# exosports/BART

Hardware: AMD Instinct MI355X
Metric: forward spectra/sec (100 layers x 1e4 wavenumbers) (higher is better)
Workload: dtype f64; 1 GPU; H2O+CO+CO2+CH4 eclipse, 100 layers x 10000 wavenumbers, 10 walkers batched per GPU per step (BASELINE config 3), opacity-table path, 27 T planes, H2-H2 CIA, 5 ray angles, toomuch 10, SURVEY 8d opacities, every step its own profile preparation; nlayers=100, nwave=10000, integ=1, cut=slant, cia_interp=spline, kappa_model=survey8d, parallelism=single GPU

## Files before the change

### bart_amd/csrc/capi.hip

```cpp
#include <cstring>
#include <stdexcept>
#include <string>

#include "../../include/bartrt.h"
#include "comm.hpp"
#include "contrib.hpp"
#include "engine.hpp"
#include "lbl.hpp"
#include "share.hpp"
#include "step.hpp"
#include "rt_launch.hpp"
#include "rtc.hpp"
#include "svc.hpp"

#include <climits>
#include <cstdio>
#include <cstdlib>

#include <sys/stat.h>
#include <unistd.h>

using namespace bartrt;

static Engine *g_eng = nullptr;
// ... 596 lines not shown
  return BARTRT_OK;
}

int bartrt_walked_end(int *walked, int cap, int *nwalkers, int *ncolumns, int *wn_per_column,
                      char *kernel, int kernel_len) {
  NEED_ENGINE();
  return guarded([&] {
    Engine *e = g_eng;
    e->want_walked = false;
    HIPCHK(hipDeviceSynchronize());
    const int n = e->walked_nwalkers, nc = e->walked_info.ncolumns;
    if (nwalkers) *nwalkers = n;
    if (ncolumns) *ncolumns = nc;
    if (wn_per_column) *wn_per_column = e->walked_info.wn_per_column;
    if (kernel && kernel_len > 0) {
      std::snprintf(kernel, (size_t)kernel_len, "%s%s%s%s", e->walked_info.kernel, e->walked_info.rtc ? " [instantiated at run time]" : "",
                    e->walked_info.prep_folded ? " [prepares its own walkers]" : "",
                    e->walked_info.window ? " [table through a moving window]" : "");
    }
    if (walked && n > 0) {
      if ((size_t)cap < (size_t)n * nc) throw std::invalid_argument("walked_end: buffer too small");
      HIPCHK(hipMemcpy(walked, e->d_walked, sizeof(int) * (size_t)n * nc, hipMemcpyDeviceToHost));
    }
    return BARTRT_OK;
  });
}

int bartrt_get_rtc_stats(int *available, int *compiled, int *from_disk, int *failed, double *compile_seconds) {
  const RtcStats st = rtc_stats();
  if (available) *available = rtc_available() ? 1 : 0;
  if (compiled) *compiled = st.compiled;
// ... 302 lines not shown
```

### bart_amd/csrc/engine.hip

```cpp
#include "engine.hpp"
#include "lbl.hpp"
#include "lds.hpp"
#include "prep.hpp"
#include "contrib.hpp"
#include "share.hpp"
#include "step.hpp"
#include "svc.hpp"

#include <algorithm>
#include <climits>
#include <cmath>
#include <cstdlib>
#include <cstring>
#include <stdexcept>

#include <sys/stat.h>
#include <unistd.h>

namespace bartrt {

EngineStream::~EngineStream() {
  for (auto e : ev) (void)hipEventDestroy(e);
  if (stream) (void)hipStreamDestroy(stream);
}
// ... 183 lines not shown
      hi_wn = 1.0 / (cfg_num(cfg, "wllow", 0) * wlfct);
    } else {
      throw IoError{"transit cfg: no spectral range (wnlow/wnhigh or wllow/wlhigh)"};
    }
    double d = cfg_num(cfg, "wndelt", 1.0) * wnfct;
    if (!(d > 0) || !(hi_wn > lo_wn)) throw IoError{"transit cfg: bad spectral sampling"};
    long n = (long)std::floor((hi_wn - lo_wn) / d + 1e-9) + 1;
    wn_full.resize(n);
    for (long i = 0; i < n; i++) wn_full[i] = lo_wn + d * (double)i;
    M = 0; Nt = 2; tgrid = {0.0, 1.0};
  }
  Wfull = (int)wn_full.size();
  lo = (int)((long)Wfull * shard_rank / shard_n);
  hi = (int)((long)Wfull * (shard_rank + 1) / shard_n);
  if (hi <= lo) throw IoError{"--shard leaves this rank without wavenumber samples"};
}

void Engine::read_geometry() {
  angles = cfg_list(cfg, "raygrid");
  if (angles.empty()) angles = {0, 20, 40, 60, 80};
  A = (int)angles.size();
  if (A > kMaxAngles) throw IoError{"raygrid: too many angles"};
  for (int a = 0; a < A; a++)
    if (angles[a] < 0 || angles[a] >= 90 || (a && angles[a] <= angles[a - 1]))
      throw IoError{"raygrid: angles must increase within [0, 90)"};
  toomuch = cfg_num(cfg, "toomuch", 20.0);
  if (!cfg_has(cfg, "gsurf") || !cfg_has(cfg, "refpress") || !cfg_has(cfg, "refradius"))
    throw IoError{"transit cfg: gsurf, refpress and refradius are required"};
  gsurf = cfg_num(cfg, "gsurf", 0);
  refpress = cfg_num(cfg, "refpress", 0) * 1e6;
// ... 230 lines not shown
  }
  pa.consts = d_prep_consts;
  if (M > kMaxMol) throw IoError{"more opacity-table molecules than the kernels are built for (16)"};
  for (int m = 0; m < M; m++) pa.opmol[m] = opmol[m];
  pa.ncia_temps = (int)cia_temp.size();
  const size_t prep_lds = sizeof(double) * prep_lds_doubles(L, S, Nt, pa.ncia_temps);
  if (prep_lds > kLdsMax)
    throw IoError{"the column's preparation does not fit in LDS: L = " + std::to_string(L) + " layers and S = " +
                  std::to_string(S) + " species need " + std::to_string(prep_lds) + " bytes of the " +
                  std::to_string(kLdsMax) + " a workgroup has"};
  pa.iH2 = iH2; pa.iHe = iHe;

  RtArgs &r = rt;
  r.L = L; r.M = M; r.Nt = Nt; r.C = C; r.A = A; r.W = Wl; r.Wfull = Wfull;
  r.kappa = d_kappa; r.cia = d_cia; r.wn = d_wn;
  r.kappa_bytes = (unsigned long long)L * Nt * M * Wl * 8ull;
  r.cia_bytes = (unsigned long long)cia_planes.size() * 8ull;
  for (int a = 0; a < A; a++) {
    double lo_a = a == 0 ? 0.0 : 0.5 * (angles[a - 1] + angles[a]);
    double hi_a = a == A - 1 ? 90.0 : 0.5 * (angles[a] + angles[a + 1]);
    double sl = std::sin(lo_a * kPI / 180.0), sh = std::sin(hi_a * kPI / 180.0);
    r.wgt[a] = kPI * (sh * sh - sl * sl);
    r.invmu[a] = 1.0 / std::cos(angles[a] * kPI / 180.0);
    r.wq[a] = r.wgt[a] * r.invmu[a];
    r.mu[a] = std::cos(angles[a] * kPI / 180.0);
  }
}

void Engine::start_workspaces() {
  if (!cfg_has(cfg, "opacityfile") && cfg_has(cfg, "linedb")) {
// ... 15 lines not shown
    }
  HIPCHK(hipMemcpy(d_prof, hp.data(), sizeof(double) * hp.size(), hipMemcpyHostToDevice));
  run(RunRequest(d_prof, 1, d_spec, rec[0].ok, stream));
  run(RunRequest(d_prof, nw, d_spec, rec[0].ok, stream));
  HIPCHK(hipStreamSynchronize(stream));
  forget_profiles();
}

void Engine::setup(const TCfg &cfg_in, int shard_rank, int shard_n) {
  cfg = cfg_in;
  read_settings();
  generate_missing_opacity_file(shard_rank);
  read_atmosphere();
  OpacityHeader oh;
  read_grid(oh, shard_rank, shard_n);
  read_geometry();
  open_device();
  upload_table(oh);
  std::vector<double> cia_planes, cia_temp;
  resample_cia(cia_planes, cia_temp);
  upload_constants(cia_planes, cia_temp);
  start_workspaces();
}

void Engine::ensure_walkers(int n) {
  if (n <= cap_walkers) return;
  int cap = std::max(n, cap_walkers * 2);
  HIPCHK(hipDeviceSynchronize());
  if (last_prof == d_prof) forget_profiles();
  pf_have_prof = nullptr;
  if (cap2) {
    rec[1].reserve((size_t)cap, L, M, C);
    cap2 = cap;
  }
  d_prof.reserve((size_t)cap * (S + 1) * L);
  rec[0].reserve((size_t)cap, L, M, C);
  d_spec.reserve((size_t)cap * W());
  d_rad.reserve((size_t)cap * L);
  if (solution == 1) {
    d_rtop.reserve((size_t)cap * L);
    d_ds.reserve((size_t)cap * chord_table_size(L));
  }
  cap_walkers = cap;
}

void Engine::ensure_second_set() {
  if (cap2 >= cap_walkers) return;
  HIPCHK(hipDeviceSynchronize());
  rec[1].reserve((size_t)cap_walkers, L, M, C);
  cap2 = cap_walkers;
}

void Engine::wait(hipStream_t st) {
  if (!sync_poll || !h_flag) { HIPCHK(hipStreamSynchronize(st)); return; }
  const unsigned int want = ++flag_seq;
  HIPCHK(hipStreamWriteValue32(st, d_flag, want, 0));
  volatile unsigned int *f = h_flag;
  long spins = 0;
  while (*f != want) {
    __builtin_ia32_pause();
    if ((++spins & 0xfffff) == 0 && hipStreamQuery(st) != hipErrorNotReady) { HIPCHK(hipStreamSynchronize(st)); break; }
  }
  __atomic_thread_fence(__ATOMIC_ACQUIRE);
}
// ... 126 lines not shown

PrepArgs Engine::prep_args(const RunRequest &rq, const RecordSet &records) {
  PrepArgs pa = prep;
  pa.nwalkers = rq.n;
  pa.prof = rq.prof;
  pa.gsurf = gsurf; pa.refradius = refradius;
  pa.scat_flag = rq.scat_flag >= 0 ? rq.scat_flag : scat_flag; pa.scat_value = scat_value;
  pa.has_cloud = has_cloud; pa.cloudtop = cloudtop;
  pa.cloud_rup = cloud_rup; pa.cloud_rdown = cloud_rdown; pa.cloud_ext = cloud_ext;
  pa.coef = records.coef; pa.idx = records.idx; pa.kstop = records.kstop;
  pa.ok = rq.ok ? rq.ok : rec[0].ok.get();
  pa.rad_out = d_rad;
  pa.over = rq.over;
  pa.rtop = solution == 1 ? d_rtop.get() : nullptr;
  pa.ds = solution == 1 ? d_ds.get() : nullptr;
  return pa;
}

static int rt_block() {
  static const int b = [] { const char *e = std::getenv("BARTRT_BLOCK"); return e ? std::atoi(e) : 64; }();
  return (b == 128 || b == 256) ? b : 64;
}

RtArgs Engine::rt_args(const RunRequest &rq, const PrepArgs &pa, const Prefetch &pf, bool eclipse_rt, bool timed) {
  const int n = rq.n, block = rt_block();
  RtArgs r = rt;
  r.nwalkers = n;
  r.nsel = rq.sel_walkers > n ? rq.sel_walkers : 0;
  if (kernel_by_local) r.Wfull = r.W;
  r.coef = pa.coef; r.idx = pa.idx; r.kstop = pa.kstop;
// ... 55 lines not shown
    r.walked_out = d_walked;
    walked_nwalkers = n;
  }
  return r;
}

void Engine::run_chunk(const RunRequest &rq) {
  const int n = rq.n;
  hipStream_t st = rq.stream;
  if (n > cap_walkers) ensure_walkers(n);
  const bool eclipse_rt = solution == 0 && !rq.lbl_fused;
  const bool plain = eclipse_rt && !lbl && !rq.d_ext && !rq.prep_hook && !rq.want_tau && !rq.want_intens;
  const bool pf_ok = plain && !rq.over;
  const Prefetch pf = plan_prefetch(pf_ok, rq);
  const bool use_have = pf.have, want_next = pf.want_next;
  const PrepArgs pa = prep_args(rq, rec[pf.bset]);
  const bool try_fold = plain && !use_have && !want_next && std::max(n, rq.sel_walkers) <= 4 && integ == 1 && cut_slant &&
                        A == 5;
  if (use_have) {
    if (rq.ok) HIPCHK(hipMemcpyAsync(rq.ok, rec[pf.bset].ok, (size_t)n, hipMemcpyDeviceToDevice, st));
  } else if (rq.prep_hook) HIPCHK(rq.prep_hook(pa, st, rq.prep_hook_ctx));
  else if (!try_fold) HIPCHK(launch_prep(pa, st));
  if (solution == 1) HIPCHK(launch_chord_table(pa, st));

  const bool timed = timing && n > 0 && rt.W > 0 && (timing_seen++ % timing_stride == 0);
  const RtArgs r = rt_args(rq, pa, pf, eclipse_rt, timed);
  if (rq.lbl_fused) lbl_rt_eclipse(*this, rq.prof, n, r, st);
  else if (solution == 1) {
    RtLaunchInfo li;
    HIPCHK(launch_transit(r, st, &li));
    if (want_walked) walked_info = li;
  }
  else {
    RtLaunchInfo li;
    bool folded = false;
    if (try_fold) HIPCHK(launch_rt_folded(r, pa, rt_block(), st, &li, &folded));
    if (!folded) {
      if (try_fold) HIPCHK(launch_prep(pa, st));
      li = RtLaunchInfo{};
      HIPCHK(launch_rt(r, rt_block(), st, &li));
    }
    if (want_walked) walked_info = li;
    if (want_next && li.prep_fused) {
      pf_have_prof = rq.next_prof; pf_have_n = rq.next_n; pf_have_buf = 1 - pf.bset;
      pf_have_stream = st; pf_have_set = pf.now;
    }
  }
  if (timed) {
    if (rq.lbl_fused) HIPCHK(hipEventRecord(ev[ev_used + 1], st));
    ev_used += 2;
  }
}

}
```

### bart_amd/csrc/engine.hpp

```cpp
#pragma once
#include <hip/hip_runtime.h>

#include <string>
#include <vector>

#include "devbuf.hpp"
#include "io.hpp"
#include "kernels.hpp"

namespace bartrt {

hipError_t launch_prep(const PrepArgs &a, hipStream_t st);
hipError_t launch_rt(const RtArgs &a, int block, hipStream_t st, RtLaunchInfo *info = nullptr);
hipError_t launch_rt_folded(const RtArgs &a, const PrepArgs &prep, int block, hipStream_t st, RtLaunchInfo *info, bool *folded);
hipError_t launch_transit(const RtArgs &a, hipStream_t st, RtLaunchInfo *info = nullptr);
hipError_t launch_chord_table(const PrepArgs &a, hipStream_t st);
hipError_t launch_grid_transpose(const double *src, double *dst, long planes, int M, int W, hipStream_t st);

int parse_integ(const std::string &v);
int resolve_share_mode(const TCfg &cfg, bool no_service);

struct TableShare;
struct StepArgs;
struct Lbl;
struct Comm;
struct CfState;

struct EngineStream {
  hipStream_t stream = nullptr;
  std::vector<hipEvent_t> ev;
  ~EngineStream();
};

struct RecordSet {
  DevBuf<double> coef;
  DevBuf<idx_t> idx;
  DevBuf<int> kstop;
  DevBuf<unsigned char> ok;
  void reserve(size_t cap, int L, int M, int C) {
    coef.reserve(cap * L * coef_stride(M, C));
    idx.reserve(cap * L * idx_stride(C));
    kstop.reserve(cap);
    ok.reserve(cap);
  }
};

struct RunRequest {
  const double *prof;
  int n;
  double *spec;
  unsigned char *ok;
  hipStream_t stream;
  bool want_tau = false;
// ... 14 lines not shown
struct Engine : EngineStream {
  TCfg cfg;
  Atm atm;
  MolInfo mol;
  int L = 0, S = 0, M = 0, Nt = 0, C = 0, A = 0;
  int Wfull = 0, lo = 0, hi = 0;
  int W() const { return hi - lo; }
  std::vector<double> wn_full, tgrid, mass, angles;
  std::vector<int> opmol;
  double toomuch = 20.0, gsurf = 0, refpress = 0, refradius = 0;
  int scat_flag = 0, iH2 = -1, iHe = -1, has_cloud = 0;
  int solution = 0;
  int integ = 0;
  bool cut_slant = false;
  bool kernel_by_local = true;
  bool cia_spline = false;
  double starrad = 0;
  double scat_value = 0, cloudtop = 0;
  double cloud_rup = 0, cloud_rdown = 0, cloud_ext = 0;
  bool transparent = false;
  int device = 0;
  const double *d_kappa = nullptr;
  DevBuf<double> kappa_own, d_cia, d_wn, d_wn_full, d_press, d_mass, d_diam;
  TableShare *kappa_share = nullptr;
  int share_mode = -1;
  DevBuf<double> d_prep_consts;
  PrepArgs prep{};
  RtArgs rt{};
  int cap_walkers = 0;
  DevBuf<double> d_prof, d_spec;
// ... 43 lines not shown
  PrepSettings pf_have_set{};
  int cap2 = 0;
  DevBuf<char> d_slog;
  StepArgs *step = nullptr;
  Lbl *lbl = nullptr;
  CfState *cf = nullptr;

  ~Engine();
  void init(int argc, const char **argv);
  void setup(const TCfg &cfg_in, int shard_rank, int shard_n);
  void read_settings();
  void generate_missing_opacity_file(int shard_rank);
  void read_atmosphere();
  void read_grid(OpacityHeader &oh, int shard_rank, int shard_n);
  void read_geometry();
  void open_device();
  void upload_table(const OpacityHeader &oh);
  void resample_cia(std::vector<double> &cia_planes, std::vector<double> &cia_temp);
  void upload_constants(const std::vector<double> &cia_planes, const std::vector<double> &cia_temp);
  void start_workspaces();
  void ensure_walkers(int n);
  void ensure_second_set();
  void ensure_pin(size_t bytes);
  void run(const RunRequest &rq);
  void run_host(const double *prof, int n, int nprof, double *spec, int nwave, unsigned char *ok);
  void run_chunks(const RunRequest &rq, int chunk, bool with_ext);
  void run_chunk(const RunRequest &rq);
  struct Prefetch;
  Prefetch plan_prefetch(bool pf_ok, const RunRequest &rq);
  PrepArgs prep_args(const RunRequest &rq, const RecordSet &records);
// ... 8 lines not shown
```

### bart_amd/csrc/kernels.hip

```cpp
#include "integ.hpp"
#include "kernels.hpp"
#include "lds.hpp"
#include "prep.hpp"

#include <cmath>
#include <cstdio>
#include <cstdlib>
#include <cstring>
#include <utility>

namespace bartrt {

template <int INTEG>
bool launch_rt_spec(const RtArgs &a, int block, hipStream_t st, KernelMode mode, bool force_window,
                    bool allow_sq, hipError_t &err, RtLaunchInfo *info, const PrepArgs *fold = nullptr);
extern template bool launch_rt_spec<0>(const RtArgs &, int, hipStream_t, KernelMode, bool, bool, hipError_t &, RtLaunchInfo *, const PrepArgs *);
extern template bool launch_rt_spec<1>(const RtArgs &, int, hipStream_t, KernelMode, bool, bool, hipError_t &, RtLaunchInfo *, const PrepArgs *);
extern template bool launch_rt_spec<2>(const RtArgs &, int, hipStream_t, KernelMode, bool, bool, hipError_t &, RtLaunchInfo *, const PrepArgs *);

__global__ __launch_bounds__(256) void prep_profiles(PrepArgs p) {
  extern __shared__ double sm[];
  prep_block(p, blockIdx.x, sm);
}

__device__ inline void block_to_work_g(int b, int nwalkers, int &tile, int &walker) {
  const int xcd = b & 7, j = b >> 3;
  walker = j % nwalkers;
  tile = (j / nwalkers) * 8 + xcd;
}

template <int AT, int MT, int CT, int INTEG>
__global__ __launch_bounds__(256) void rt_eclipse(RtArgs p) {
  extern __shared__ double smem[];
  const int A = AT > 0 ? AT : p.A;
  const int M = MT >= 0 ? MT : p.M;
  const int C = CT >= 0 ? CT : p.C;
// ... 131 lines not shown
}

hipError_t launch_grid_transpose(const double *src, double *dst, long planes, int M, int W, hipStream_t st) {
  if (planes <= 0 || M <= 0 || W <= 0) return hipSuccess;
  const int ntiles = (W + 63) / 64;
  if (planes * ntiles > 0x7fffffffL) return hipErrorInvalidValue;
  hipLaunchKernelGGL(grid_transpose, dim3((unsigned)(planes * ntiles)), dim3(64), 0, st, src, dst, M, W, ntiles);
  return hipGetLastError();
}

hipError_t launch_prep(const PrepArgs &a, hipStream_t st) {
  if (a.nwalkers <= 0) return hipSuccess;
  const size_t sh = sizeof(double) * prep_lds_doubles(a.L, a.S, a.Nt, a.ncia_temps);
  static size_t allowed = kLdsDefault;
  if (hipError_t e = allow_lds(prep_profiles, sh, allowed); e != hipSuccess) return e;
  hipLaunchKernelGGL(prep_profiles, dim3(a.nwalkers), dim3(256), sh, st, a);
  return hipGetLastError();
}

template <int AT, int INTEG>
static hipError_t launch_rt_t(const RtArgs &a, int block, int nblocks, hipStream_t st) {
  const size_t sh = sizeof(double) * ((size_t)a.L * coef_stride(a.M, a.C) +
                                      (INTEG == kIntegSimpson ? simpson_lds_doubles(a.L) : 0)) +
                    sizeof(idx_t) * (size_t)a.L * idx_stride(a.C);
  static size_t allowed = 64 * 1024;
  if (sh > allowed) {
    if (sh > 160 * 1024) return hipErrorInvalidValue;
    hipError_t e = hipFuncSetAttribute(reinterpret_cast<const void *>(rt_eclipse<AT, -1, -1, INTEG>),
                                       hipFuncAttributeMaxDynamicSharedMemorySize, (int)sh);
    if (e != hipSuccess) return e;
    allowed = sh;
// ... 76 lines not shown
```

### bart_amd/csrc/kernels.hpp

```cpp
#pragma once
#ifndef __HIPCC_RTC__
#include <hip/hip_runtime.h>
#include <hip/hip_ext.h>
#include <cstdint>
#else
typedef struct ihipEvent_t *hipEvent_t;
namespace std {
template <class T, T v> struct integral_constant { static constexpr T value = v; using value_type = T; constexpr operator T() const { return v; } };
using true_type = integral_constant<bool, true>;
using false_type = integral_constant<bool, false>;
template <bool B, class T, class F> struct conditional { using type = T; };
template <class T, class F> struct conditional<false, T, F> { using type = F; };
template <bool B, class T, class F> using conditional_t = typename conditional<B, T, F>::type;
}
#endif

#define BARTRT_MC_LIST(X) \
  X(1, 0) X(1, 1) X(1, 2) X(2, 0) X(2, 1) X(2, 2) X(3, 0) X(3, 1) X(3, 2) X(4, 0) X(4, 1) X(4, 2) \
  X(5, 0) X(5, 1) X(5, 2) X(6, 0) X(6, 1) X(6, 2)                                                 \
  X(1, 4) X(2, 4) X(3, 4) X(4, 4) X(5, 4) X(6, 4)
#define BARTRT_QADJ_LIST(X) BARTRT_MC_LIST(X)
#define BARTRT_EXT_C_LIST(X) X(0) X(1) X(2) X(4)

#define BARTRT_RT_LAUNCH(kernel, grid, block, sh, st, args) \
// ... 102 lines not shown
  int ref_ib;
  double ref_f;
  double ref_lnp;
  double gsurf, refradius;
  int scat_flag, iH2, iHe, has_cloud;
  double scat_value, cloudtop;
  double cloud_rup, cloud_rdown, cloud_ext;
  const double *over;
  double *coef;
  idx_t *idx;
  int *kstop;
  unsigned char *ok;
  double *rad_out;
  double *rtop;
  double *ds;
};

struct RtArgs {
  int L, M, Nt, C, A, W, nwalkers, ntiles;
  int nsel;
  int Wfull;
  const double *kappa;
  const double *cia;
  unsigned long long kappa_bytes, cia_bytes;
  int window;
  const double *ext;
  const double *wn;
  const double *coef;
  const idx_t *idx;
  const int *kstop;
// ... 8 lines not shown
  double thr[kMaxAngles];
  double thrb[kMaxAngles];
  int drank[kMaxAngles];
  void *slog;
  double *spec;
  double *tau_out;
  int *last_out;
  double *intens_out;
  int *walked_out;
  const double *rtop, *ds;
  double inv_starrad2;
  int transparent;
  hipEvent_t ev_start, ev_stop;
  int nprep;
  PrepArgs prep_next;
};
__host__ __device__ inline int prep_slots(int nprep) { return (nprep + 7) / 8 * 8; }

inline void slant_thresholds(RtArgs &r) {
  for (int a = 0; a < r.A; a++) {
    const double im = r.invmu[a];
    double t = r.toomuch / im;
    if (!(t == t) || t > 1.7e308 || t < 0.0) { r.thr[a] = t < 0.0 ? -1.0 : 1.7976931348623157e308; continue; }
    for (int it = 0; it < 64 && t * im > r.toomuch; it++) t = __builtin_nextafter(t, 0.0);
    for (int it = 0; it < 64; it++) {
      const double up = __builtin_nextafter(t, 1.7976931348623157e308);
      if (up == t || up * im > r.toomuch) break;
      t = up;
    }
    r.thr[a] = t;
// ... 6 lines not shown
    r.drank[a] = rk;
  }
}
inline size_t slant_log_bytes(int nwalkers, int ntiles, int block, int A) {
  return (size_t)nwalkers * (size_t)ntiles * (size_t)block * (size_t)A * 20u;
}

struct RtLaunchInfo {
  const char *kernel = "";
  int wn_per_column = 64;
  int ncolumns = 0;
  bool prep_fused = false;
  bool prep_folded = false;
  bool rtc = false;
  bool window = false;
};

#ifndef __HIPCC_RTC__
enum class KernelMode { kDefault, kGeneric, kMono, kMonoOcc, kMonoIlp, kSplit, kQuad, kOcto, kHexa, kR32, kAdj8, kAdj16 };
KernelMode rt_kernel_mode();
#endif

constexpr double kExpShift = 6755399441055744.0;
constexpr double kExpMin = -708.0;

__device__ __forceinline__ double exp_scale(double p, double shifted) {
  const int hi = __double2hiint(p) + (__double2loint(shifted) << 20);
  return __hiloint2double(hi, __double2loint(p));
}

// ... 5 lines not shown
  double p = 2.5110037605963777e-08;
  p = fma(p, r, 2.763263963904103e-07);
  p = fma(p, r, 2.755724091857897e-06);
  p = fma(p, r, 2.4801485482328494e-05);
  p = fma(p, r, 0.00019841269890047113);
  p = fma(p, r, 0.0013888888952314775);
  p = fma(p, r, 0.008333333333319601);
  p = fma(p, r, 0.0416666666664881);
  p = fma(p, r, 0.1666666666666668);
  p = fma(p, r, 0.5000000000000019);
  p = fma(p, r, 1.0);
  p = fma(p, r, 1.0);
  return exp_scale(p, t);
}

__device__ __forceinline__ double rcp_core(double d) {
  double y = __builtin_amdgcn_rcp(d);
  double e = fma(-d, y, 1.0);
  y = fma(y, e, y);
  e = fma(-d, y, 1.0);
  return fma(y, e, y);
}
__device__ __forceinline__ double rcp_n1(double d) {
  const double y = __builtin_amdgcn_rcp(d);
  return fma(y, fma(-d, y, 1.0), y);
}

template <int N>
__device__ __forceinline__ void exp_rt_n(const double (&x)[N], double (&out)[N]) {
  double t[N], r[N], q[N];
// ... 115 lines not shown
```

### bart_amd/csrc/prep.hpp

```cpp
#pragma once
#include "kernels.hpp"

#ifdef BARTRT_PHASE_CLOCK
extern __device__ unsigned long long g_phase_clock[32];
#define BARTRT_PHASE(n) do { if (blockIdx.x == 0 && threadIdx.x == 0) g_phase_clock[n] = __builtin_amdgcn_s_memrealtime(); } while (0)
#else
#define BARTRT_PHASE(n) do {} while (0)
#endif

namespace bartrt {

__device__ inline int bracket_dev(const double *g, const double *ginv, int n, double t) {
  if (n <= 2) return 0;
  double x = (t - g[0]) * ginv[0];
  int j = x > 0.0 ? (x < (double)(n - 2) ? (int)x : n - 2) : 0;
  const double a = g[j], b = g[j + 1];
  if ((j == n - 2 || b > t) && (j == 0 || a <= t)) return j;
  while (j < n - 2 && g[j + 1] <= t) j++;
  while (j > 0 && g[j] > t) j--;
  return j;
}


__host__ __device__ inline size_t prep_lds_doubles(int L, int S, int Nt, int ncia_temps) {
// ... 202 lines not shown
  if (threadIdx.x == 0) {
    int ks = L - 1;
    if (has_cloud) {
      for (int k = 0; k < L; k++)
        if (sPress[L - 1 - k] >= cloudtop) { ks = k | kDeckBit; break; }
    }
    if (fold.kstop) *fold.kstop = ks;
    if (fold.global) {
      p.kstop[w] = ks;
      if (p.ok) p.ok[w] = bad ? 0 : 1;
    }
  }
  BARTRT_PHASE(11);
}

__device__ inline void prep_block(const PrepArgs &p, int w, double *sm, const PrepFold fold = PrepFold{}) {
  const int L = p.L, S = p.S;
  BARTRT_PHASE(7);
  stage2_to_lds(prep_lds_profile(sm, L), p.prof + (size_t)w * (S + 1) * L, (S + 1) * L,
                prep_lds_consts(sm, L, S), p.consts, 2 * L + S + 2 * p.Nt + 2 * p.ncia_temps,
                threadIdx.x, blockDim.x);
  prep_body(p, w, sm, p.over ? p.over + (size_t)3 * w : nullptr, fold);
}

}
```

### bart_amd/csrc/rt_eclipse_s1s.hpp

```cpp
#pragma once
#include "integ.hpp"
#include "kernels.hpp"
#include "rt_eclipse_s1.hpp"

#ifndef __HIPCC_RTC__
#include <type_traits>
#endif

namespace bartrt {

#ifndef BARTRT_FLAG_CLAMP
#define BARTRT_FLAG_CLAMP 1
#endif
template <int A>
__device__ __forceinline__ double alive_flags(const RtArgs &p, double tm, double (&m)[A]) {
  double n = 0.0;
#if BARTRT_FLAG_CLAMP
  const double tb = tm * -4.149515568880993e180;
#pragma unroll
  for (int a = 0; a < A; a++) {
    asm("v_add_f64 %0, %1, %2 clamp" : "=v"(m[a]) : "v"(tb), "s"(p.thrb[a]));
    n += m[a];
  }
#else
#pragma unroll
  for (int a = 0; a < A; a++) {
    m[a] = tm <= p.thr[a] ? 1.0 : 0.0;
    n += m[a];
  }
#endif
  return n;
}

template <int AT, int MT, int CT, bool SQ, int SCHED = 1, bool EXT = false, bool OUT = false>
__global__ __launch_bounds__(256) __attribute__((amdgpu_waves_per_eu(OUT ? 1 : 2, BARTRT_WPE)))
void rt_eclipse_simpson_slant(RtArgs p) {
  extern __shared__ double smem[];
  constexpr int A = AT, M = MT, C = CT;
  constexpr int NC = 4 + 2 * M + 2 * C, NI = 1 + C, NLD = 2 * M + 2 * C;
  constexpr int NR = NLD + (EXT ? 1 : 0) > 0 ? NLD + (EXT ? 1 : 0) : 1;
  constexpr int AE = SQ ? A - 1 : A;
  constexpr int kBlk = 6;
  static_assert(kBlk - 2 <= kSimpsonPad, "the radius table's overrun entries");
  const int L = p.L, W = p.W;
  int bid = blockIdx.x;
  if (p.nprep > 0) {
    if (bid < p.nprep) { prep_block(p.prep_next, bid, smem); return; }
    bid -= prep_slots(p.nprep);
    if (bid < 0) return;
  }
  int tile, w;
  block_to_work(bid, p.nwalkers, tile, w);
  if (tile >= p.ntiles) return;

  double *sC = smem;
  idx_t *sI = reinterpret_cast<idx_t *>(smem + (size_t)L * NC);
  double *sWw = smem + (size_t)L * NC + (size_t)L * NI;
  const double *sW = sWw;
  stage2_to_lds(sC, p.coef + (size_t)w * L * NC, L * NC, sI, p.idx + (size_t)w * L * NI, L * NI, threadIdx.x,
                blockDim.x);
  const int kraw = p.kstop[w], kend = kstop_layer(kraw);
  const bool deck_on = kstop_deck(kraw);
  __syncthreads();
  simpson_radius_table(sWw, sC, NC, L, kend, threadIdx.x, blockDim.x);
  __syncthreads();

  const int i = tile * blockDim.x + threadIdx.x;
  const bool valid = i < W;
  const unsigned ii = valid ? (unsigned)i : (unsigned)(W - 1);
  const double nu = p.wn[ii];
  const double bnum = 2.0 * kH * nu * nu * nu * kLS * kLS;
  const double nu4 = (nu * nu) * (nu * nu);
  const TableLoader<M, C> tab(p, ii, sI);
  const double *extw = EXT ? p.ext + (size_t)w * L * W + ii : nullptr;
  auto load_layer = [&](int k, double (&r)[NR]) {
    tab.load(k, r);
    if constexpr (EXT) r[NLD] = extw[(size_t)(L - 1 - k) * W];
  };
  const double tcap = tau_cap(p, A);
  const int kcut = kend < L - 2 ? kend : L - 2;
  double thr_max = p.thr[0];
#pragma unroll
  for (int a = 1; a < A; a++) thr_max = p.thr[a] > thr_max ? p.thr[a] : thr_max;

  double s_even = 0.0, eprev = 0.0, e2 = 0.0;
  double x1 = 0.0, h0 = 0.0, r0 = 1.0, tm = 0.0;
  [[maybe_unused]] int out_last = 0;
  [[maybe_unused]] double out_tau = 0.0;
  double y1[A], y2[A], P0[A], P1[A];
#pragma unroll
  for (int a = 0; a < A; a++) { y1[a] = y2[a] = P0[a] = P1[a] = 0.0; }
  const unsigned nth = blockDim.x;
// ... 52 lines not shown
    double m[A];
    const double nnow = alive_flags<A>(p, tm, m);
    if constexpr (OUT) {
      if (p.tau_out && valid && inr && tm <= thr_max) {
        p.tau_out[(size_t)i * L + k] = tau;
        out_last = k;
        out_tau = tau;
      }
    }
    if constexpr (MASKED) {
#pragma unroll
      for (int a = 0; a < A; a++) m[a] = inr ? m[a] : 0.0;
    }
    if constexpr (!(FIRST && J == 0)) log_event(nnow, k - 1);
    const double tcl = fmin(tau, tcap);
    double xs[AE + 1], ex[AE + 1], y[A];
    xs[AE] = fmin(cf[1] * nu, 700.0);
#pragma unroll
    for (int a = 0; a < AE; a++) xs[a] = -tcl * p.invmu[a];
    exp_rt_n<AE + 1>(xs, ex);
    const double B = bnum * rcp_n1(ex[AE] - 1.0);
#pragma unroll
    for (int a = 0; a < AE; a++) y[a] = B * ex[a];
    if (SQ) y[A - 1] = (B * ex[0]) * ex[0];
    if constexpr (FIRST && J == 0) {
#pragma unroll
      for (int a = 0; a < A; a++) y1[a] = y[a];
    } else {
      double h1 = tau - x1;
      if constexpr (MASKED) h1 = inr ? h1 : 1.0;
      double w0, w1, w2, r1 = 1.0;
      if constexpr (FIRST && J == 1) {
        w0 = 0.0; w1 = w2 = 0.5 * h1;
      } else {
        r1 = rcp_n1(h1);
        const double hs = h0 + h1, s6 = hs * (1.0 / 6.0);
// ... 186 lines not shown
      }
    }
    F = fast_ok ? F_fast : F;
  }
  if constexpr (OUT) {
    if (p.tau_out && valid) {
      for (int kk = out_last + 1; kk < L; kk++) p.tau_out[(size_t)i * L + kk] = out_tau;
      p.last_out[i] = out_last;
    }
  }
  if (valid) p.spec[(size_t)w * W + i] = F;
  if (p.walked_out && threadIdx.x == 0)
    p.walked_out[(size_t)w * p.ntiles + tile] = (kw < kend + 1 ? kw : kend + 1);
}


}
```

### bart_amd/csrc/rt_eclipse_slant_ilp.hip

```cpp
#include "rt_launch.hpp"

#define BARTRT_SLANT(MM, CC)                                                                                                \
  BARTRT_K(simpson_slant, 5, MM, CC, true, slant_sched(MM, CC, 1)) BARTRT_K(simpson_slant, 5, MM, CC, false, slant_sched(MM, CC, 1)) \
  BARTRT_K(fast, 5, MM, CC, true, 0, 1, false, true) BARTRT_K(fast, 5, MM, CC, false, 0, 1, false, true)                    \
  BARTRT_K(fast, 5, MM, CC, true, 2, 1, false, true) BARTRT_K(fast, 5, MM, CC, false, 2, 1, false, true)
#define BARTRT_SLANT_OUT(MM, CC) BARTRT_K(simpson_slant, 5, MM, CC, false, 0, false, true)
#define BARTRT_SLANT_EXT(CC)                                                                              \
  BARTRT_K(simpson_slant, 5, 0, CC, true, 1, true) BARTRT_K(simpson_slant, 5, 0, CC, false, 1, true)      \
  BARTRT_K(fast, 5, 0, CC, true, 0, 1, true, true) BARTRT_K(fast, 5, 0, CC, false, 0, 1, true, true)
#define BARTRT_UNIT slant_ilp
#define BARTRT_UNIT_KERNELS BARTRT_MC_LIST(BARTRT_SLANT) BARTRT_MC_LIST(BARTRT_SLANT_OUT) BARTRT_EXT_C_LIST(BARTRT_SLANT_EXT)
#include "rt_eclipse_unit.inc"
```

### bart_amd/csrc/rt_launch.hpp

```cpp
#pragma once
#include "rt_eclipse.hpp"
#include "rtc.hpp"

#include <cmath>
#include <cstdio>
#include <cstdlib>
#include <string>
#include <utility>

namespace bartrt {

constexpr long kQuadMaxColumns = 640, kQuadMaxColumnsSimpson = 480;
constexpr long kQuadRaysMaxColumns = 80;
constexpr long kOctoRaysMaxColumns = 40;
constexpr int kFoldMaxWorkgroups = 512;
constexpr long kOctoMaxColumns = 400;
constexpr long kSplitMinColumns = 1025, kSplitMaxColumns = 1300;
constexpr long kIlpMaxColumns = 20000;

enum KernelVariant { kVarSingle = 0, kVarRows4 = 4, kVarRows8 = 8, kVarRows16 = 16, kVarRows32 = 32, kVarAdj8 = 108, kVarAdj16 = 116 };
struct KernelChoice { long max_columns; int variant, fallback; };
constexpr long kAllColumns = 0x7fffffffffffffffL;
#include "kernel_table.inc"
inline const KernelChoice &slant_simpson_choice(int M, long columns) {
// ... 6 lines not shown
}
inline const char *kernel_variant_name(int v) {
  switch (v) {
    case kVarRows4: return "rows4"; case kVarRows8: return "rows8"; case kVarRows16: return "rows16"; case kVarRows32: return "rows32";
    case kVarAdj8: return "adj8"; case kVarAdj16: return "adj16"; default: return "single";
  }
}

enum class KFamily { Fast, Simpson, SimpsonSlant, Quad, Qadj, Split };
struct KernelId {
  KFamily family;
  int A, M, C;
  bool sq;
  int integ = 0, sched = 0, rows = 0;
  bool ext = false, slant = false, out = false, rays = false, allr = false;
};
constexpr KernelId fast_id(int A, int M, int C, bool sq, int integ, int sched = 0, bool ext = false, bool slant = false) {
  return {KFamily::Fast, A, M, C, sq, integ, sched, 0, ext, slant, false, false, false};
}
constexpr KernelId split_id(int A, int M, int C, bool sq, int integ) {
  return {KFamily::Split, A, M, C, sq, integ, 0, 0, false, false, false, false, false};
}
constexpr KernelId quad_id(int A, int M, int C, bool sq, int rows, int integ, bool rays = false, bool allr = false) {
  return {KFamily::Quad, A, M, C, sq, integ, 0, rows, false, false, false, rays, allr};
}
constexpr KernelId simpson_id(int A, int M, int C, bool sq, int sched = 0, bool ext = false) {
  return {KFamily::Simpson, A, M, C, sq, 0, sched, 0, ext, false, false, false, false};
}
constexpr KernelId simpson_slant_id(int A, int M, int C, bool sq, int sched = 1, bool ext = false, bool out = false) {
  return {KFamily::SimpsonSlant, A, M, C, sq, 0, sched, 0, ext, false, out, false, false};
}
constexpr KernelId qadj_id(int A, int M, int C, bool sq, int rows) {
  return {KFamily::Qadj, A, M, C, sq, 0, 0, rows, false, false, false, false, false};
}
constexpr unsigned long long kernel_key(const KernelId &k) {
  return (unsigned long long)k.family | (unsigned long long)(k.A & 255) << 4 | (unsigned long long)(k.M & 255) << 12 |
         (unsigned long long)(k.C & 255) << 20 | (unsigned long long)(k.rows & 255) << 28 | (unsigned long long)(k.integ & 15) << 36 |
         (unsigned long long)(k.sched & 15) << 40 | (unsigned long long)k.sq << 44 | (unsigned long long)k.ext << 45 |
         (unsigned long long)k.slant << 46 | (unsigned long long)k.out << 47 | (unsigned long long)k.rays << 48 |
         (unsigned long long)k.allr << 49;
}

inline std::string kernel_expr(const KernelId &k) {
  const auto tf = [](bool b) { return b ? "true" : "false"; };
  char s[160];
  switch (k.family) {
    case KFamily::Fast:
      std::snprintf(s, sizeof s, "rt_eclipse_fast<%d, %d, %d, %s, %d, %d, %s, %s>", k.A, k.M, k.C, tf(k.sq), k.integ, k.sched, tf(k.ext), tf(k.slant));
      break;
    case KFamily::Simpson:
      std::snprintf(s, sizeof s, "rt_eclipse_simpson<%d, %d, %d, %s, %d, %s>", k.A, k.M, k.C, tf(k.sq), k.sched, tf(k.ext));
      break;
    case KFamily::SimpsonSlant:
      std::snprintf(s, sizeof s, "rt_eclipse_simpson_slant<%d, %d, %d, %s, %d, %s, %s>", k.A, k.M, k.C, tf(k.sq), k.sched, tf(k.ext), tf(k.out));
      break;
    case KFamily::Quad:
      std::snprintf(s, sizeof s, "rt_eclipse_quad<%d, %d, %d, %s, %d, %d, %s, %s>", k.A, k.M, k.C, tf(k.sq), k.rows, k.integ, tf(k.rays), tf(k.allr));
      break;
    case KFamily::Qadj:
      std::snprintf(s, sizeof s, "rt_eclipse_qadj<%d, %d, %d, %s, %d>", k.A, k.M, k.C, tf(k.sq), k.rows);
      break;
    case KFamily::Split:
      std::snprintf(s, sizeof s, "rt_eclipse_split<%d, %d, %d, %s, %d>", k.A, k.M, k.C, tf(k.sq), k.integ);
      break;
  }
  return s;
}

// ... 164 lines not shown
  return true;
}

struct LpGeom { RtArgs b; int wn, ncolumns, nwg; size_t lds; bool folds; };
inline LpGeom lp_geom(const SpecLaunch &c, int rows, int wn) {
  LpGeom g{c.b, wn, 0, 0, 0, false};
  g.b.ntiles = (c.a.W + 4 * wn - 1) / (4 * wn);
  g.ncolumns = 4 * g.b.ntiles;
  g.nwg = c.workgroups(g.b.ntiles);
  g.lds = c.sh + c.shp + (rows >= 16 ? sizeof(double) * (size_t)c.a.L : 0);
  g.folds = c.fold && g.lds + c.sh_fold <= 64 * 1024 && (g.b.ntiles + 7) / 8 * 8 * c.nsel + c.pslots <= kFoldMaxWorkgroups;
  if (g.folds) { g.b.nprep = -1; g.b.prep_next = *c.fold; g.lds += c.sh_fold; }
  return g;
}

inline bool launch_single_wave(const SpecLaunch &c, const KernelId &id, const RtArgs &args) {
  return launch_kernel(c, id, c.workgroups(args.ntiles), c.block, c.sh + c.shp, args) && c.launched(kernel_label(id), c.block, args.ntiles);
}
inline bool launch_layer_parallel(const SpecLaunch &c, const KernelId &id, const LpGeom &g) {
  return launch_kernel(c, id, g.nwg, 256, g.lds, g.b) && c.launched(kernel_label(id), g.wn, g.ncolumns, g.folds, g.b.window != 0);
}

template <int INTEG>
bool launch_form_ext(const SpecLaunch &c) {
  const RtArgs &b = c.b;
  const KernelId id = b.cut_slant ? (INTEG == kIntegSimpson ? simpson_slant_id(5, b.M, b.C, c.sq, 1, true) : fast_id(5, b.M, b.C, c.sq, INTEG, 1, true, true))
                                  : (INTEG == kIntegSimpson ? simpson_id(5, b.M, b.C, c.sq, 1, true) : fast_id(5, b.M, b.C, c.sq, INTEG, 1, true));
  return launch_kernel(c, id, c.nblocks, c.block, c.sh, b) && c.launched(kernel_label(id), c.block, b.ntiles);
}

// ... 20 lines not shown
bool launch_form_quad_allr(const SpecLaunch &c, const LpGeom &g, int rows) {
  static_assert(INTEG == kIntegSimpson, "the all-rays form: rule 1");
  return launch_layer_parallel(c, quad_id(5, g.b.M, g.b.C, c.sq, rows, INTEG, false, true), g);
}

template <int INTEG>
bool launch_form_quad_rays(const SpecLaunch &c, int rows) {
  static_assert(INTEG != kIntegSimpson, "the one-ray-per-lane form: rules 0 / 2");
  const LpGeom g = lp_geom(c, rows, 64 / rows / 5);
  return launch_layer_parallel(c, quad_id(5, g.b.M, g.b.C, false, rows, INTEG, true), g);
}

template <int INTEG>
bool launch_form_slant(const SpecLaunch &c) {
  const RtArgs &b = c.b;
  return launch_single_wave(c, INTEG == kIntegSimpson ? simpson_slant_id(5, b.M, b.C, c.sq, slant_sched(b.M, b.C, 1))
                                                      : fast_id(5, b.M, b.C, c.sq, INTEG, 1, false, true),
                            b);
}

template <int INTEG>
bool launch_form_quad(const SpecLaunch &c, int rows) {
  const LpGeom g = lp_geom(c, rows, 64 / rows);
  return launch_layer_parallel(c, quad_id(5, g.b.M, g.b.C, c.sq, rows, INTEG), g);
}

template <int INTEG>
bool launch_form_split(const SpecLaunch &c) {
  RtArgs b = c.b;
  b.ntiles = (b.W + 63) / 64;
// ... 91 lines not shown
```

Before: 95540 spectra/s.

## Factorise the Planck exponential into per-tile base and per-offset tables

Replaces the per-sample exp(c·ν/T) in the Simpson slant eclipse kernel with a product of two factors. One is a per-layer exponential at the tile's base wavenumber, kept in LDS. The other is a per-layer, per-offset exponential table that the prep kernel computes in extra workgroups and the RT kernel reads through buffer loads. This removes one exp per layer and sample from the hot loop, at the cost of an extra global load, extra LDS, and extra prep work. It is gated on a uniformly sampled grid check, an environment override, and an LDS occupancy check.

```diff
diff --git a/bart_amd/csrc/capi.hip b/bart_amd/csrc/capi.hip
--- a/bart_amd/csrc/capi.hip
+++ b/bart_amd/csrc/capi.hip
@@ -634,7 +634,8 @@
     if (ncolumns) *ncolumns = nc;
     if (wn_per_column) *wn_per_column = e->walked_info.wn_per_column;
     if (kernel && kernel_len > 0) {
-      std::snprintf(kernel, (size_t)kernel_len, "%s%s%s%s", e->walked_info.kernel, e->walked_info.rtc ? " [instantiated at run time]" : "",
+      std::snprintf(kernel, (size_t)kernel_len, "%s%s%s%s%s", e->walked_info.kernel, e->walked_info.planck_factor ? " [Planck exponential factorised]" : "",
+                    e->walked_info.rtc ? " [instantiated at run time]" : "",
                     e->walked_info.prep_folded ? " [prepares its own walkers]" : "",
                     e->walked_info.window ? " [table through a moving window]" : "");
     }
diff --git a/bart_amd/csrc/engine.hip b/bart_amd/csrc/engine.hip
--- a/bart_amd/csrc/engine.hip
+++ b/bart_amd/csrc/engine.hip
@@ -221,6 +221,37 @@
   lo = (int)((long)Wfull * shard_rank / shard_n);
   hi = (int)((long)Wfull * (shard_rank + 1) / shard_n);
   if (hi <= lo) throw IoError{"--shard leaves this rank without wavenumber samples"};
+}
+
+void Engine::plan_planck_factor() {
+  planck_factor = false;
+  std::string v;
+  if (const char *e = std::getenv("BARTRT_PLANCK")) v = e;
+  if (!v.empty() && v != "direct" && v != "factor") throw IoError{"BARTRT_PLANCK: '" + v + "' is neither direct nor factor"};
+  std::string why;
+  double dev = 0.0, amax = 0.0;
+  if (M < 1 || tgrid.empty() || !(tgrid.front() > 0)) why = "the engine has no opacity table";
+  else if (Wfull < 2) why = "the grid has a single sample";
+  else {
+    const double nu0 = wn_full.front(), dnu = (wn_full.back() - nu0) / (double)(Wfull - 1);
+    amax = (kH * kLS / kKB) / tgrid.front();
+    if (!(dnu > 0) || !(nu0 >= 0)) why = "the grid does not ascend from a non-negative wavenumber";
+    else {
+      for (int i = 0; i < Wfull; i++) {
+        const int g = i & ~(kPlanckTile - 1);
+        const long double model = (long double)std::fma((double)g, dnu, nu0) + (long double)(dnu * (double)(i - g));
+        dev = std::max(dev, (double)fabsl((long double)wn_full[i] - model));
+      }
+      if (!(dev * amax <= 1e-13)) {
+        char t[200];
+        std::snprintf(t, sizeof t, "the grid is not uniformly sampled: it deviates by %.3g cm-1, %.3g in the Planck exponent "
+                      "at the table's lowest temperature (limit 1e-13)", dev, dev * amax);
+        why = t;
+      } else { planck_nu0 = nu0; planck_dnu = dnu; }
+    }
+  }
+  if (v == "factor" && !why.empty()) throw IoError{"BARTRT_PLANCK=factor: " + why};
+  planck_factor = why.empty() && v != "direct";
 }
 
 void Engine::read_geometry() {
@@ -481,6 +512,7 @@
   RtArgs &r = rt;
   r.L = L; r.M = M; r.Nt = Nt; r.C = C; r.A = A; r.W = Wl; r.Wfull = Wfull;
   r.kappa = d_kappa; r.cia = d_cia; r.wn = d_wn;
+  r.pf_e1 = nullptr; r.pf_nu0 = planck_nu0; r.pf_dnu = planck_dnu; r.pf_lo = lo;
   r.kappa_bytes = (unsigned long long)L * Nt * M * Wl * 8ull;
   r.cia_bytes = (unsigned long long)cia_planes.size() * 8ull;
   for (int a = 0; a < A; a++) {
@@ -526,6 +558,7 @@
   read_atmosphere();
   OpacityHeader oh;
   read_grid(oh, shard_rank, shard_n);
+  plan_planck_factor();
   read_geometry();
   open_device();
   upload_table(oh);
@@ -543,10 +576,12 @@
   pf_have_prof = nullptr;
   if (cap2) {
     rec[1].reserve((size_t)cap, L, M, C);
+    if (planck_factor) rec[1].reserve_e1((size_t)cap, L);
     cap2 = cap;
   }
   d_prof.reserve((size_t)cap * (S + 1) * L);
   rec[0].reserve((size_t)cap, L, M, C);
+  if (planck_factor) rec[0].reserve_e1((size_t)cap, L);
   d_spec.reserve((size_t)cap * W());
   d_rad.reserve((size_t)cap * L);
   if (solution == 1) {
@@ -560,6 +595,7 @@
   if (cap2 >= cap_walkers) return;
   HIPCHK(hipDeviceSynchronize());
   rec[1].reserve((size_t)cap_walkers, L, M, C);
+  if (planck_factor) rec[1].reserve_e1((size_t)cap_walkers, L);
   cap2 = cap_walkers;
 }
 
@@ -716,6 +752,9 @@
   pa.over = rq.over;
   pa.rtop = solution == 1 ? d_rtop.get() : nullptr;
   pa.ds = solution == 1 ? d_ds.get() : nullptr;
+  const bool pf = planck_factor && solution == 0 && integ == 1 && cut_slant && A == 5 && records.e1;
+  pa.e1 = pf ? records.e1.get() : nullptr;
+  pa.e1_dnu = planck_dnu;
   return pa;
 }
 
@@ -801,17 +840,23 @@
   const bool pf_ok = plain && !rq.over;
   const Prefetch pf = plan_prefetch(pf_ok, rq);
   const bool use_have = pf.have, want_next = pf.want_next;
-  const PrepArgs pa = prep_args(rq, rec[pf.bset]);
+  RecordSet &records = rec[pf.bset];
+  const PrepArgs pa = prep_args(rq, records);
   const bool try_fold = plain && !use_have && !want_next && std::max(n, rq.sel_walkers) <= 4 && integ == 1 && cut_slant &&
                         A == 5;
   if (use_have) {
     if (rq.ok) HIPCHK(hipMemcpyAsync(rq.ok, rec[pf.bset].ok, (size_t)n, hipMemcpyDeviceToDevice, st));
-  } else if (rq.prep_hook) HIPCHK(rq.prep_hook(pa, st, rq.prep_hook_ctx));
-  else if (!try_fold) HIPCHK(launch_prep(pa, st));
+  } else if (rq.prep_hook) {
+    HIPCHK(rq.prep_hook(pa, st, rq.prep_hook_ctx));
+    records.e1_dnu = 0.0;
+  } else if (!try_fold) {
+    HIPCHK(launch_prep(pa, st));
+    records.e1_dnu = pa.e1 ? pa.e1_dnu : 0.0;
+  }
   if (solution == 1) HIPCHK(launch_chord_table(pa, st));
 
   const bool timed = timing && n > 0 && rt.W > 0 && (timing_seen++ % timing_stride == 0);
-  const RtArgs r = rt_args(rq, pa, pf, eclipse_rt, timed);
+  RtArgs r = rt_args(rq, pa, pf, eclipse_rt, timed);
   if (rq.lbl_fused) lbl_rt_eclipse(*this, rq.prof, n, r, st);
   else if (solution == 1) {
     RtLaunchInfo li;
@@ -823,12 +868,17 @@
     bool folded = false;
     if (try_fold) HIPCHK(launch_rt_folded(r, pa, rt_block(), st, &li, &folded));
     if (!folded) {
-      if (try_fold) HIPCHK(launch_prep(pa, st));
+      if (try_fold) {
+        HIPCHK(launch_prep(pa, st));
+        records.e1_dnu = pa.e1 ? pa.e1_dnu : 0.0;
+      }
+      if (eclipse_rt && !lbl && !rq.d_ext && pa.e1 && records.e1_dnu == planck_dnu && planck_dnu > 0) r.pf_e1 = pa.e1;
       li = RtLaunchInfo{};
       HIPCHK(launch_rt(r, rt_block(), st, &li));
     }
     if (want_walked) walked_info = li;
     if (want_next && li.prep_fused) {
+      rec[1 - pf.bset].e1_dnu = 0.0;
       pf_have_prof = rq.next_prof; pf_have_n = rq.next_n; pf_have_buf = 1 - pf.bset;
       pf_have_stream = st; pf_have_set = pf.now;
     }
diff --git a/bart_amd/csrc/engine.hpp b/bart_amd/csrc/engine.hpp
--- a/bart_amd/csrc/engine.hpp
+++ b/bart_amd/csrc/engine.hpp
@@ -37,6 +37,9 @@
   DevBuf<idx_t> idx;
   DevBuf<int> kstop;
   DevBuf<unsigned char> ok;
+  DevBuf<double> e1;
+  double e1_dnu = 0.0;
+  void reserve_e1(size_t cap, int L) { e1.reserve(cap * L * kPlanckTile); e1_dnu = 0.0; }
   void reserve(size_t cap, int L, int M, int C) {
     coef.reserve(cap * L * coef_stride(M, C));
     idx.reserve(cap * L * idx_stride(C));
@@ -81,6 +84,8 @@
   int integ = 0;
   bool cut_slant = false;
   bool kernel_by_local = true;
+  bool planck_factor = false;
+  double planck_nu0 = 0, planck_dnu = 0;
   bool cia_spline = false;
   double starrad = 0;
   double scat_value = 0, cloudtop = 0;
@@ -154,6 +159,7 @@
   void read_atmosphere();
   void read_grid(OpacityHeader &oh, int shard_rank, int shard_n);
   void read_geometry();
+  void plan_planck_factor();
   void open_device();
   void upload_table(const OpacityHeader &oh);
   void resample_cia(std::vector<double> &cia_planes, std::vector<double> &cia_temp);
diff --git a/bart_amd/csrc/kernels.hip b/bart_amd/csrc/kernels.hip
--- a/bart_amd/csrc/kernels.hip
+++ b/bart_amd/csrc/kernels.hip
@@ -20,6 +20,7 @@
 
 __global__ __launch_bounds__(256) void prep_profiles(PrepArgs p) {
   extern __shared__ double sm[];
+  if ((int)blockIdx.x >= p.nwalkers) { planck_e1_block(p, (int)blockIdx.x - p.nwalkers); return; }
   prep_block(p, blockIdx.x, sm);
 }
 
@@ -181,7 +182,8 @@
   const size_t sh = sizeof(double) * prep_lds_doubles(a.L, a.S, a.Nt, a.ncia_temps);
   static size_t allowed = kLdsDefault;
   if (hipError_t e = allow_lds(prep_profiles, sh, allowed); e != hipSuccess) return e;
-  hipLaunchKernelGGL(prep_profiles, dim3(a.nwalkers), dim3(256), sh, st, a);
+  const int ne1 = a.e1 ? a.nwalkers * planck_e1_blocks(a.L) : 0;
+  hipLaunchKernelGGL(prep_profiles, dim3(a.nwalkers + ne1), dim3(256), sh, st, a);
   return hipGetLastError();
 }
 
diff --git a/bart_amd/csrc/kernels.hpp b/bart_amd/csrc/kernels.hpp
--- a/bart_amd/csrc/kernels.hpp
+++ b/bart_amd/csrc/kernels.hpp
@@ -140,6 +140,8 @@
   double *rad_out;
   double *rtop;
   double *ds;
+  double *e1;
+  double e1_dnu;
 };
 
 struct RtArgs {
@@ -178,6 +180,9 @@
   hipEvent_t ev_start, ev_stop;
   int nprep;
   PrepArgs prep_next;
+  const double *pf_e1;
+  double pf_nu0, pf_dnu;
+  int pf_lo;
 };
 __host__ __device__ inline int prep_slots(int nprep) { return (nprep + 7) / 8 * 8; }
 
@@ -214,6 +219,7 @@
   bool prep_folded = false;
   bool rtc = false;
   bool window = false;
+  bool planck_factor = false;
 };
 
 #ifndef __HIPCC_RTC__
@@ -249,6 +255,9 @@
   return exp_scale(p, t);
 }
 
+constexpr double kExp700 = 1.0142320547350045e304;
+constexpr int kPlanckTile = 64;
+
 __device__ __forceinline__ double rcp_core(double d) {
   double y = __builtin_amdgcn_rcp(d);
   double e = fma(-d, y, 1.0);
diff --git a/bart_amd/csrc/prep.hpp b/bart_amd/csrc/prep.hpp
--- a/bart_amd/csrc/prep.hpp
+++ b/bart_amd/csrc/prep.hpp
@@ -240,6 +240,20 @@
   BARTRT_PHASE(11);
 }
 
+__host__ __device__ inline int planck_e1_blocks(int L) { return (L * kPlanckTile + 1023) / 1024; }
+__device__ inline void planck_e1_block(const PrepArgs &p, int e) {
+  const int nb = planck_e1_blocks(p.L), w = e / nb, part = e - w * nb;
+  const int n = p.L * kPlanckTile, end = (part + 1) * 1024 < n ? (part + 1) * 1024 : n;
+  const double *T = p.prof + (size_t)w * (p.S + 1) * p.L;
+  double *out = p.e1 + (size_t)w * n;
+  for (int t = part * 1024 + (int)threadIdx.x; t < end; t += (int)blockDim.x) {
+    const int k = t / kPlanckTile, j = t % kPlanckTile;
+    const double invT = 1.0 / T[p.L - 1 - k];
+    const double a = (kH * kLS / kKB) * invT;
+    out[t] = exp_core(fmin(fmax(a * (p.e1_dnu * (double)j), 0.0), 700.0));
+  }
+}
+
 __device__ inline void prep_block(const PrepArgs &p, int w, double *sm, const PrepFold fold = PrepFold{}) {
   const int L = p.L, S = p.S;
   BARTRT_PHASE(7);
diff --git a/bart_amd/csrc/rt_eclipse_s1s.hpp b/bart_amd/csrc/rt_eclipse_s1s.hpp
--- a/bart_amd/csrc/rt_eclipse_s1s.hpp
+++ b/bart_amd/csrc/rt_eclipse_s1s.hpp
@@ -32,13 +32,14 @@
   return n;
 }
 
-template <int AT, int MT, int CT, bool SQ, int SCHED = 1, bool EXT = false, bool OUT = false>
-__global__ __launch_bounds__(256) __attribute__((amdgpu_waves_per_eu(OUT ? 1 : 2, BARTRT_WPE)))
-void rt_eclipse_simpson_slant(RtArgs p) {
+template <int AT, int MT, int CT, bool SQ, int SCHED, bool EXT, bool OUT, bool PF>
+__device__ __forceinline__ void simpson_slant_walk(const RtArgs &p) {
   extern __shared__ double smem[];
+  static_assert(!(PF && (EXT || OUT)), "the factorised Planck exponential: the plain build only");
   constexpr int A = AT, M = MT, C = CT;
   constexpr int NC = 4 + 2 * M + 2 * C, NI = 1 + C, NLD = 2 * M + 2 * C;
-  constexpr int NR = NLD + (EXT ? 1 : 0) > 0 ? NLD + (EXT ? 1 : 0) : 1;
+  constexpr int NX = (EXT || PF) ? 1 : 0;
+  constexpr int NR = NLD + NX > 0 ? NLD + NX : 1;
   constexpr int AE = SQ ? A - 1 : A;
   constexpr int kBlk = 6;
   static_assert(kBlk - 2 <= kSimpsonPad, "the radius table's overrun entries");
@@ -63,6 +64,16 @@
   const bool deck_on = kstop_deck(kraw);
   __syncthreads();
   simpson_radius_table(sWw, sC, NC, L, kend, threadIdx.x, blockDim.x);
+  double *sE0 = sWw + 4 * (size_t)(L + kSimpsonPad);
+  if constexpr (PF) {
+    const int g = (p.pf_lo + tile * (int)blockDim.x) & ~(kPlanckTile - 1);
+    const double nug0 = fma((double)g, p.pf_dnu, p.pf_nu0), nug1 = fma((double)(g + kPlanckTile), p.pf_dnu, p.pf_nu0);
+    for (int k = threadIdx.x; k < L; k += blockDim.x) {
+      const double a = sC[k * NC + 1];
+      sE0[2 * k] = exp_core(fmin(fmax(a * nug0, 0.0), 700.0));
+      sE0[2 * k + 1] = exp_core(fmin(fmax(a * nug1, 0.0), 700.0));
+    }
+  }
   __syncthreads();
 
   const int i = tile * blockDim.x + threadIdx.x;
@@ -73,9 +84,16 @@
   const double nu4 = (nu * nu) * (nu * nu);
   const TableLoader<M, C> tab(p, ii, sI);
   const double *extw = EXT ? p.ext + (size_t)w * L * W + ii : nullptr;
+  const int gi = PF ? p.pf_lo + (int)ii : 0;
+  const unsigned e1_vo = (unsigned)(gi & (kPlanckTile - 1)) * 8u;
+  const double *e0l = sE0 + (PF && (gi >> 6) != ((p.pf_lo + tile * (int)blockDim.x) >> 6) ? 1 : 0);
+  const auto rs_e1 = __builtin_amdgcn_make_buffer_rsrc(
+      const_cast<double *>(PF ? p.pf_e1 + (size_t)w * L * kPlanckTile : nullptr), 0, PF ? L * kPlanckTile * 8 : 0, 0x00020000);
   auto load_layer = [&](int k, double (&r)[NR]) {
     tab.load(k, r);
     if constexpr (EXT) r[NLD] = extw[(size_t)(L - 1 - k) * W];
+    if constexpr (PF)
+      r[NLD] = __builtin_bit_cast(double, (v2u_t)__builtin_amdgcn_raw_buffer_load_b64(rs_e1, (int)e1_vo, k * (kPlanckTile * 8), 0));
   };
   const double tcap = tau_cap(p, A);
   const int kcut = kend < L - 2 ? kend : L - 2;
@@ -158,12 +176,16 @@
     }
     if constexpr (!(FIRST && J == 0)) log_event(nnow, k - 1);
     const double tcl = fmin(tau, tcap);
-    double xs[AE + 1], ex[AE + 1], y[A];
-    xs[AE] = fmin(cf[1] * nu, 700.0);
+    constexpr int NE = PF ? AE : AE + 1;
+    double xs[NE], ex[NE], y[A];
+    if constexpr (!PF) xs[AE] = fmin(cf[1] * nu, 700.0);
 #pragma unroll
     for (int a = 0; a < AE; a++) xs[a] = -tcl * p.invmu[a];
-    exp_rt_n<AE + 1>(xs, ex);
-    const double B = bnum * rcp_n1(ex[AE] - 1.0);
+    exp_rt_n<NE>(xs, ex);
+    double EB;
+    if constexpr (PF) EB = fmin(e0l[2 * (MASKED ? (k < kend ? k : kend) : k)] * r[NLD], kExp700);
+    else EB = ex[AE];
+    const double B = bnum * rcp_n1(EB - 1.0);
 #pragma unroll
     for (int a = 0; a < AE; a++) y[a] = B * ex[a];
     if (SQ) y[A - 1] = (B * ex[0]) * ex[0];
@@ -380,5 +402,17 @@
     p.walked_out[(size_t)w * p.ntiles + tile] = (kw < kend + 1 ? kw : kend + 1);
 }
 
-
+template <int AT, int MT, int CT, bool SQ, int SCHED = 1, bool EXT = false, bool OUT = false>
+__global__ __launch_bounds__(256) __attribute__((amdgpu_waves_per_eu(OUT ? 1 : 2, BARTRT_WPE)))
+void rt_eclipse_simpson_slant(RtArgs p) {
+  simpson_slant_walk<AT, MT, CT, SQ, SCHED, EXT, OUT, false>(p);
 }
+
+template <int AT, int MT, int CT, bool SQ, int SCHED = 1>
+__global__ __launch_bounds__(256) __attribute__((amdgpu_waves_per_eu(2, BARTRT_WPE)))
+void rt_eclipse_simpson_slant_pf(RtArgs p) {
+  simpson_slant_walk<AT, MT, CT, SQ, SCHED, false, false, true>(p);
+}
+
+
+}
diff --git a/bart_amd/csrc/rt_eclipse_slant_ilp.hip b/bart_amd/csrc/rt_eclipse_slant_ilp.hip
--- a/bart_amd/csrc/rt_eclipse_slant_ilp.hip
+++ b/bart_amd/csrc/rt_eclipse_slant_ilp.hip
@@ -4,10 +4,12 @@
   BARTRT_K(simpson_slant, 5, MM, CC, true, slant_sched(MM, CC, 1)) BARTRT_K(simpson_slant, 5, MM, CC, false, slant_sched(MM, CC, 1)) \
   BARTRT_K(fast, 5, MM, CC, true, 0, 1, false, true) BARTRT_K(fast, 5, MM, CC, false, 0, 1, false, true)                    \
   BARTRT_K(fast, 5, MM, CC, true, 2, 1, false, true) BARTRT_K(fast, 5, MM, CC, false, 2, 1, false, true)
+#define BARTRT_SLANT_PF(MM, CC)                                                                                             \
+  BARTRT_K(simpson_slant_pf, 5, MM, CC, true, slant_sched(MM, CC, 1)) BARTRT_K(simpson_slant_pf, 5, MM, CC, false, slant_sched(MM, CC, 1))
 #define BARTRT_SLANT_OUT(MM, CC) BARTRT_K(simpson_slant, 5, MM, CC, false, 0, false, true)
 #define BARTRT_SLANT_EXT(CC)                                                                              \
   BARTRT_K(simpson_slant, 5, 0, CC, true, 1, true) BARTRT_K(simpson_slant, 5, 0, CC, false, 1, true)      \
   BARTRT_K(fast, 5, 0, CC, true, 0, 1, true, true) BARTRT_K(fast, 5, 0, CC, false, 0, 1, true, true)
 #define BARTRT_UNIT slant_ilp
-#define BARTRT_UNIT_KERNELS BARTRT_MC_LIST(BARTRT_SLANT) BARTRT_MC_LIST(BARTRT_SLANT_OUT) BARTRT_EXT_C_LIST(BARTRT_SLANT_EXT)
+#define BARTRT_UNIT_KERNELS BARTRT_MC_LIST(BARTRT_SLANT) BARTRT_MC_LIST(BARTRT_SLANT_PF) BARTRT_MC_LIST(BARTRT_SLANT_OUT) BARTRT_EXT_C_LIST(BARTRT_SLANT_EXT)
 #include "rt_eclipse_unit.inc"
diff --git a/bart_amd/csrc/rt_launch.hpp b/bart_amd/csrc/rt_launch.hpp
--- a/bart_amd/csrc/rt_launch.hpp
+++ b/bart_amd/csrc/rt_launch.hpp
@@ -44,6 +44,7 @@
   bool sq;
   int integ = 0, sched = 0, rows = 0;
   bool ext = false, slant = false, out = false, rays = false, allr = false;
+  bool pf = false;
 };
 constexpr KernelId fast_id(int A, int M, int C, bool sq, int integ, int sched = 0, bool ext = false, bool slant = false) {
   return {KFamily::Fast, A, M, C, sq, integ, sched, 0, ext, slant, false, false, false};
@@ -59,6 +60,9 @@
 }
 constexpr KernelId simpson_slant_id(int A, int M, int C, bool sq, int sched = 1, bool ext = false, bool out = false) {
   return {KFamily::SimpsonSlant, A, M, C, sq, 0, sched, 0, ext, false, out, false, false};
+}
+constexpr KernelId simpson_slant_pf_id(int A, int M, int C, bool sq, int sched = 1) {
+  return {KFamily::SimpsonSlant, A, M, C, sq, 0, sched, 0, false, false, false, false, false, true};
 }
 constexpr KernelId qadj_id(int A, int M, int C, bool sq, int rows) {
   return {KFamily::Qadj, A, M, C, sq, 0, 0, rows, false, false, false, false, false};
@@ -68,7 +72,7 @@
          (unsigned long long)(k.C & 255) << 20 | (unsigned long long)(k.rows & 255) << 28 | (unsigned long long)(k.integ & 15) << 36 |
          (unsigned long long)(k.sched & 15) << 40 | (unsigned long long)k.sq << 44 | (unsigned long long)k.ext << 45 |
          (unsigned long long)k.slant << 46 | (unsigned long long)k.out << 47 | (unsigned long long)k.rays << 48 |
-         (unsigned long long)k.allr << 49;
+         (unsigned long long)k.allr << 49 | (unsigned long long)k.pf << 50;
 }
 
 inline std::string kernel_expr(const KernelId &k) {
@@ -82,6 +86,7 @@
       std::snprintf(s, sizeof s, "rt_eclipse_simpson<%d, %d, %d, %s, %d, %s>", k.A, k.M, k.C, tf(k.sq), k.sched, tf(k.ext));
       break;
     case KFamily::SimpsonSlant:
+      if (k.pf) { std::snprintf(s, sizeof s, "rt_eclipse_simpson_slant_pf<%d, %d, %d, %s, %d>", k.A, k.M, k.C, tf(k.sq), k.sched); break; }
       std::snprintf(s, sizeof s, "rt_eclipse_simpson_slant<%d, %d, %d, %s, %d, %s, %s>", k.A, k.M, k.C, tf(k.sq), k.sched, tf(k.ext), tf(k.out));
       break;
     case KFamily::Quad:
@@ -276,6 +281,15 @@
   return g;
 }
 
+inline int single_wave_workgroups_per_cu(size_t lds) {
+  const size_t granule = 1280, alloc = (lds + 8 + granule - 1) / granule * granule;
+  const size_t n = alloc ? 160 * 1024 / alloc : 8;
+  return n < 8 ? (int)n : 8;
+}
+inline bool planck_factor_fits(size_t lds_direct, size_t lds_factor) {
+  return lds_factor <= 64 * 1024 && single_wave_workgroups_per_cu(lds_factor) >= single_wave_workgroups_per_cu(lds_direct);
+}
+
 inline bool launch_single_wave(const SpecLaunch &c, const KernelId &id, const RtArgs &args) {
   return launch_kernel(c, id, c.workgroups(args.ntiles), c.block, c.sh + c.shp, args) && c.launched(kernel_label(id), c.block, args.ntiles);
 }
@@ -326,6 +340,16 @@
 template <int INTEG>
 bool launch_form_slant(const SpecLaunch &c) {
   const RtArgs &b = c.b;
+  if constexpr (INTEG == kIntegSimpson) {
+    const size_t lds = c.sh + c.shp, e0 = sizeof(double) * 2 * (size_t)b.L;
+    if (b.pf_e1 && c.block == 64 && planck_factor_fits(lds, lds + e0)) {
+      const KernelId id = simpson_slant_pf_id(5, b.M, b.C, c.sq, slant_sched(b.M, b.C, 1));
+      if (launch_kernel(c, id, c.workgroups(b.ntiles), c.block, lds + e0, b)) {
+        if (c.info) c.info->planck_factor = true;
+        return c.launched(kernel_label(id), c.block, b.ntiles);
+      }
+    }
+  }
   return launch_single_wave(c, INTEG == kIntegSimpson ? simpson_slant_id(5, b.M, b.C, c.sq, slant_sched(b.M, b.C, 1))
                                                       : fast_id(5, b.M, b.C, c.sq, INTEG, 1, false, true),
                             b);
```

After: 90290 spectra/s. -5.5%, worse.
